# kangzf/GraphEmbedding

Hardware: AMD Instinct MI355X
Metric: graph-pairs/sec (Siamese fwd+bwd), AIDS700 all-pairs @ 1/2/4/8 MI355X (higher is better)
Workload: dtype f32; 1 GPU; AIDS700nef all-pairs (700 graphs, 490,000 ordered pairs), default 5-layer Siamese GCN-NTN, dropout 0.1; global_batch=490000, n_max=10, d_in=29, records=f32 Â, 896 B/pair, order=class, inputs=records resident in HBM, parallelism=dp1, adam=in the gradient reduction's launch (sg_train_step)

## Files before the change

graphembedding_amd/csrc/sg_fast.hip:

```cpp
#include <type_traits>

#include "sg_plan.h"
#include "sg_mfma.h"

int sg_num_cus();

namespace {

using namespace sgk;

constexpr int FH1 = 32, FH2 = 16, FK = 10;
constexpr int TS1 = 36;
constexpr int TS2 = 20;
constexpr int W1S = 20;
constexpr int W1TS = 36;
__device__ __forceinline__ void mfma_fence() { __builtin_amdgcn_sched_barrier(0); }
constexpr int MAXW = 8;

struct FastArgs {
  const uint8_t *recs;
  const int32_t *order;
  const int32_t *cls;
  float cw[4];
  int xw[8];
  int xw_even;
  int64_t n_pairs;
  int64_t pair_offset;
  int rw4h;
  int rec_bf16;
  const float *params;
  const float *y_stats;
  float *s_out;
  float *slab;
  float *ntn;
  uint32_t key;
  const uint64_t *seed_dev;
  const float *ad_bp;
  float *ad_out;
  float ad_lr, ad_b1, ad_b2, ad_wd;
  uint32_t thr0, thr1, thr2, thr4;
  float ik0, ik1, ik2, ik4;
  float yeta;
  float inv_batch;
  int d_in, n_params;
  int shared_floats, wave_floats;
  int oW0, ob0, oW1, ob1, oWd, obd, oW, oV, oU, obn;
  int oWa;
  int src_store, G;
  const float *sadj;
  const int32_t *stypes, *sn, *spairs;
  int64_t grid_base;
  const float *slabels;
  int32_t *status;
};

template <int D>
__device__ __forceinline__ uint4 fast_store_word(const FastArgs &A, int p, int w4, int lane) {
  int g0, g1;
  if (A.spairs) {
    g0 = A.spairs[2 * (int64_t)p];
    g1 = A.spairs[2 * (int64_t)p + 1];
  } else {
    const int64_t q = A.grid_base + p;
    g0 = (int)(q / A.G);
    g1 = (int)(q - (int64_t)g0 * A.G);
  }
  const bool ok = (unsigned)g0 < (unsigned)A.G && (unsigned)g1 < (unsigned)A.G;
  if (!ok && lane == 0 && A.status) atomicExch(A.status, (int32_t)SG_ERR_ARG);
  constexpr int NN = D * D;
  uint32_t v[4];
#pragma unroll
  for (int k = 0; k < 4; ++k) {
    const int w = 4 * w4 + k;
    uint32_t x = 0u;
    if (ok) {
      if (w < 2 * NN) {
        const int s = w >= NN;
        x = __float_as_uint(A.sadj[(size_t)(s ? g1 : g0) * NN + (w - s * NN)]);
      } else if (w < 2 * NN + 2 * D) {
        const int t = w - 2 * NN, s = t >= D;
        x = (uint32_t)A.stypes[(size_t)(s ? g1 : g0) * D + (t - s * D)];
      } else if (w == 2 * NN + 2 * D) {
        x = (uint32_t)A.sn[g0];
      } else if (w == 2 * NN + 2 * D + 1) {
        x = (uint32_t)A.sn[g1];
      } else if (w == 2 * NN + 2 * D + 2) {
        x = __float_as_uint(A.slabels ? A.slabels[p] : 0.f);
      } else if (w == 2 * NN + 2 * D + 3) {
        x = (uint32_t)p;
      }
    }
    v[k] = x;
  }
  return uint4{v[0], v[1], v[2], v[3]};
}

constexpr int WAS = 17;

template <int D, bool AVG = false, bool ATT = false>
struct FastLds {
  static constexpr int DN = AVG ? FH2 : D, WR = AVG ? 16 : 12, VS = 34;
  static_assert(2 * DN <= VS, "V row");
  static constexpr int RW = 2 * D * D + 2 * D + 4;
  static constexpr int REC = 0;
  static constexpr int TILE = REC + RW;
  static constexpr int X = TILE + 2 * 16 * TS1;
  static constexpr int GE = X + 48;
  static constexpr int TMP = GE + 32;
  static constexpr int GU = TMP + 32;
  static constexpr int GT = GU + 32;
  static int wave_floats(int, bool bwd) {
    return bwd ? GT + 2 * 16 * TS2 : X + 48 + (AVG ? 32 : 0) + (ATT ? 64 : 0);
  }
  static int shared_floats(int d_in) {
    return (d_in + 1) * FH1 + 2 * DN * FK * WR + FK * VS + FH1 * W1S + FH2 * W1TS +
           2 * 3 * 64 * 4 + (ATT ? FH2 * WAS : 0);
  }
};


template <int D, bool AVG = false, bool ATT = false>
struct FlushSlots {
  static constexpr int DN = FastLds<D, AVG>::DN, RN = (DN + 3) / 4;
  static constexpr int NWS = AVG ? 0 : RN * DN, NVS = AVG ? 0 : 2 * RN;
  static constexpr int NS = 8 + 16 + NWS + NVS + 3 + 5 + (ATT ? 4 : 0);
};

template <int D, bool AVG, bool ATT>
__device__ __forceinline__ int fast_param(const FastArgs &A, int s, int l) {
  constexpr int DN = FastLds<D, AVG>::DN, RN = (DN + 3) / 4;
  constexpr int NWS = FlushSlots<D, AVG>::NWS, NVS = FlushSlots<D, AVG>::NVS;
  const int g = l >> 4, j = l & 15;
  if (s < 8) return A.oW1 + (16 * (s >> 2) + 4 * g + (s & 3)) * FH2 + j;
  s -= 8;
  if (s < 16) {
    const int ty = 16 * (s >> 3) + 4 * g + (s & 3);
    return ty < A.d_in ? A.oW0 + ty * FH1 + 16 * ((s >> 2) & 1) + j : -1;
  }
  s -= 16;
  if (s < NWS) {
    const int a = 4 * (s / DN) + g, b = s % DN;
    return (a < DN && j < FK) ? A.oW + (a * DN + b) * FK + j : -1;
  }
  s -= NWS;
  if (s < NVS) {
    const int a = 4 * (s % RN) + g;
    return (a < DN && j < FK) ? A.oV + j * 2 * DN + (s >= RN ? DN : 0) + a : -1;
  }
  s -= NVS;
  switch (s) {
    case 0: return (!AVG && g == 0 && j < FK) ? A.obn + j : -1;
    case 1: return (g == 0 && j < FK) ? A.oU + j : -1;
    case 2: return l == 0 ? A.n_params : -1;
    case 3: return g == 0 ? A.ob0 + j : -1;
    case 4: return g == 0 ? A.ob0 + 16 + j : -1;
    case 5: return g == 0 ? A.ob1 + j : -1;
    case 6: return (!AVG && g == 0) ? A.oWd + j : -1;
    case 7: return (!AVG && l == 0) ? A.obd : -1;
    default: break;
  }
  s -= 8;
  return (ATT && s < 4) ? A.oWa + (4 * s + g) * FH2 + j : -1;
}

__device__ __forceinline__ f2 pfma(f2 a, f2 b, f2 c) { return __builtin_elementwise_fma(a, b, c); }

__device__ __forceinline__ float sg_tanh(float z) {
  return 1.f - 2.f * __builtin_amdgcn_rcpf(__expf(2.f * z) + 1.f);
}
__device__ __forceinline__ float sg_sigmoid(float z) {
  return __builtin_amdgcn_rcpf(1.f + __expf(-z));
}

__device__ __forceinline__ void xsum_pair(float &a, float &b) {
  const auto r = __builtin_amdgcn_permlane16_swap(__float_as_uint(a), __float_as_uint(b), false,
                                                  false);
  const float s = __uint_as_float(r[0]) + __uint_as_float(r[1]);
  const auto q = __builtin_amdgcn_permlane32_swap(__float_as_uint(s), __float_as_uint(s), false,
                                                  false);
  const float t = __uint_as_float(q[0]) + __uint_as_float(q[1]);
  const auto z = __builtin_amdgcn_permlane16_swap(__float_as_uint(t), __float_as_uint(t), false,
                                                  false);
  a = __uint_as_float(z[0]);
  b = __uint_as_float(z[1]);
}

#ifdef SG_FAST_TIMING
constexpr int kTimeWaves = 4096;
__device__ unsigned long long sg_fast_times[kTimeWaves * 5];
#define SG_STAMP(slot, val)                                                        \
  do {                                                                             \
    const int tw_ = blockIdx.x * (blockDim.x >> 6) + (threadIdx.x >> 6);            \
    if ((threadIdx.x & 63) == 0 && tw_ < kTimeWaves) sg_fast_times[tw_ * 5 + (slot)] = (val); \
  } while (0)
#else
#define SG_STAMP(slot, val) do {} while (0)
#endif

template <int D, bool BWD, bool ALIGNED, bool INTENDED, bool AVG, bool SRC, bool ATT>
// ... 77 lines not shown
        for (int c = 0; c < 4; ++c)
          if (wt[c] > 0.f && fr[c] > bf) {
            bf = fr[c];
            bc = c;
          }
        wc[bc] += 1;
        fr[bc] = -2.f;
      }
      if (align) {
#pragma unroll
        for (int c = 0; c < 4; ++c) wc[c] *= 2;
      }
      int cum = 0;
#pragma unroll
      for (int c = 0; c < 4; ++c) {
        if (cwave < 0 && pos < cum + wc[c]) {
          const int nc = cb[c + 1] - cb[c];
          cwave = c;
          const int q = nc / wc[c], r = nc - q * wc[c];
          if (q >= 64 && A.xw_even) {
            const int k = pos - cum;
            if ((uint64_t)(uint32_t)nc * (uint32_t)wc[c] < (1ull << 32)) {
              cs0 = cb[c] + __builtin_amdgcn_readfirstlane(
                                (int)(((uint32_t)nc * (uint32_t)k) / (uint32_t)wc[c]));
              cs1 = cb[c] + __builtin_amdgcn_readfirstlane(
                                (int)(((uint32_t)nc * (uint32_t)(k + 1)) / (uint32_t)wc[c]));
            } else {
              cs0 = cb[c] + (int)((int64_t)nc * k / wc[c]);
              cs1 = cb[c] + (int)((int64_t)nc * (k + 1) / wc[c]);
            }
          } else if (q >= 64) {
            auto F = [&](int x) -> int64_t {
              const int xb = (x >> 3) & 7;
              int64_t pre = 0, tot = 0;
#pragma unroll
              for (int i = 0; i < 8; ++i) {
                tot += A.xw[i];
                pre += i < xb ? A.xw[i] : 0;
              }
              return (int64_t)(x >> 6) * 8 * tot + 8 * pre + (int64_t)(x & 7) * A.xw[xb];
            };
            const int64_t f0 = F(cum), span = F(cum + wc[c]) - f0;
            cs0 = cb[c] + (int)((int64_t)nc * (F(pos) - f0) / span);
            cs1 = cb[c] + (int)((int64_t)nc * (F(pos + 1) - f0) / span);
          } else {
            int k;
            if (align) {
              k = ((gw & 4) == 0 ? 0 : wc[c] >> 1) + ((pos - cum) >> 1);
            } else {
              auto old_below = [](int x) -> int { return (x >> 3) * 4 + min(x & 7, 4); };
              const int end = cum + wc[c];
              const int n_old = old_below(end) - old_below(cum);
              k = (gw & 4) == 0 ? old_below(gw) - old_below(cum)
                                : n_old + (gw - old_below(gw)) - (cum - old_below(cum));
            }
            cs0 = cb[c] + k * q + min(k, r);
            cs1 = cs0 + q + (k < r ? 1 : 0);
          }
        }
        cum += wc[c];
      }
    }
  }
  const bool cls_mode = cwave >= 0;
  const int qend = cls_mode ? cs1 : npairs;
  auto slot_of = [&](int r) -> int {
    if (cls_mode) return cs0 + r;
    return r * stride + ((ord != nullptr && (r & 1)) ? stride - 1 - gw : gw);
  };
  auto load_ord = [&](int r0) -> int {
    const int s = slot_of(r0 + l);
    return s < qend ? ord[s] : 0;
  };
  auto ord_at = [&](int v, int lane) -> int {
    const int x = __builtin_amdgcn_readlane(v, lane);
    return x < 0 ? 0 : (x >= npairs ? npairs - 1 : x);
  };
  int ordA = 0, ordB = 0;
  if (ord) {
    ordA = load_ord(0);
    ordB = load_ord(64);
  }

  float *sW0 = smem;
  float *sWa = sW0 + (d_in + 1) * FH1;
  float *sWb = sWa + DN * FK * WR;
  float *sV = sWb + DN * FK * WR;
  float *sW1 = sV + FK * VS;
  float *sW1T = sW1 + FH1 * W1S;
  uint4 *sW1B = (uint4 *)(sW1T + FH2 * W1TS);
  float *sWat = (float *)(sW1B + 2 * 3 * 64);
  float *W = smem + A.shared_floats + wv * A.wave_floats;
  float *sRec = W + L::REC;
  float *sT = W + L::TILE;
  float *sX = W + L::X;

#pragma unroll
  for (int k = 0; k < 8; ++k) {
    const int i = k * bdx + tid;
    if (i < nprm) stg[i] = stv[k];
  }
  for (int i = 8 * bdx + tid; i < nprm; i += bdx) stg[i] = prm[i];
  int q = slot_of(0);
  int p = (ord && q < qend) ? ord_at(ordA, 0) : q;
  const int rw4h = A.rw4h;
  constexpr int ADJ4 = D * D / 4;
  uint4 pre[NREC];
#pragma unroll
  for (int c = 0; c < NREC; ++c) {
    const int w4 = l + 64 * c;
    pre[c] = (q < qend && w4 < rw4h)
                 ? (SRC ? fast_store_word<D>(A, p, w4, l)
                                : ((const uint4 *)(A.recs + (size_t)p * (size_t)rw4h * 16u))[w4])
                 : uint4{0u, 0u, 0u, 0u};
  }
  __syncthreads();
  if (ad_blk) {
    double ss = 0.0;
    for (int i = l; i < nprm; i += 64) {
      const double t = (double)stg[i];
      ss += t * t;
    }
#pragma unroll
    for (int o = 32; o > 0; o >>= 1) ss += __shfl_xor(ss, o);
    if (l == 0) {
      A.ad_out[0] = A.ad_lr * sqrtf(1.f - ad_b2p) / (1.f - ad_b1p);
      A.ad_out[1] = ad_b1p * A.ad_b1;
      A.ad_out[2] = ad_b2p * A.ad_b2;
      A.ad_out[3] = (float)((double)A.ad_wd * 0.5 * ss);
    }
  }
  auto wa_src = [&](int i, bool tr) -> float {
    const int x = i / (FK * WR), rem = i - x * FK * WR, k = rem / WR, y = rem - k * WR;
    return y < DN ? stg[A.oW + (tr ? (y * DN + x) : (x * DN + y)) * FK + k] : 0.f;
  };
  auto v_src = [&](int i) -> float {
    const int k = i / VS, c = i - k * VS;
    return c < 2 * DN ? stg[A.oV + k * 2 * DN + c] : 0.f;
  };
  constexpr int NWA = DN * FK * WR, KWA = (NWA + 511) / 512, NVT = FK * VS, KV = (NVT + 511) / 512;
  static_assert(FH1 * FH2 == 512, "one W1 element per thread of a 512-thread block");
  const int nw0 = (d_in + 1) * FH1;
  if (bdx == 512 && nw0 <= 3 * 512) {
    float r0[3], ra[KWA], rb[KWA], rv[KV];
#pragma unroll
    for (int k = 0; k < 3; ++k) {
      const int i = min(tid + 512 * k, nw0 - 1);
      r0[k] = i < d_in * FH1 ? stg[A.oW0 + i] : 0.f;
    }
#pragma unroll
    for (int k = 0; k < KWA; ++k) {
      const int i = min(tid + 512 * k, NWA - 1);
      ra[k] = wa_src(i, false);
      rb[k] = wa_src(i, true);
    }
#pragma unroll
    for (int k = 0; k < KV; ++k) rv[k] = v_src(min(tid + 512 * k, NVT - 1));
    const float w1 = stg[A.oW1 + tid];
#pragma unroll
    for (int k = 0; k < 3; ++k)
      if (tid + 512 * k < nw0) sW0[tid + 512 * k] = r0[k] * (A.ik0 * A.ik1);
#pragma unroll
    for (int k = 0; k < KWA; ++k)
      if (tid + 512 * k < NWA) {
        sWa[tid + 512 * k] = ra[k];
        sWb[tid + 512 * k] = rb[k];
      }
#pragma unroll
    for (int k = 0; k < KV; ++k)
      if (tid + 512 * k < NVT) sV[tid + 512 * k] = rv[k];
    sW1[(tid / FH2) * W1S + tid % FH2] = w1 * A.ik1;
    sW1T[(tid % FH2) * W1TS + tid / FH2] = w1;
  } else {
    for (int i = tid; i < nw0; i += bdx)
      sW0[i] = i < d_in * FH1 ? stg[A.oW0 + i] * (A.ik0 * A.ik1) : 0.f;
    for (int i = tid; i < NWA; i += bdx) {
      sWa[i] = wa_src(i, false);
      sWb[i] = wa_src(i, true);
    }
    for (int i = tid; i < NVT; i += bdx) sV[i] = v_src(i);
    for (int i = tid; i < FH1 * FH2; i += bdx) {
      const float w = stg[A.oW1 + i];
      sW1[(i / FH2) * W1S + i % FH2] = w * A.ik1;
      sW1T[(i % FH2) * W1TS + i / FH2] = w;
    }
  }
  for (int i = tid; i < 2 * 3 * 64; i += blockDim.x) {
    const int t = i / 192, term = (i / 64) % 3, ln = i & 63;
    const int f = 16 * t + (ln & 15), k0 = 4 * (ln >> 4);
    const float *wr = stg + A.oW1 + f * FH2 + k0;
    uint32_t h01, m01, l01, h23, m23, l23;
    split3(wr[0] * A.ik1, wr[1] * A.ik1, h01, m01, l01);
    split3(wr[2] * A.ik1, wr[3] * A.ik1, h23, m23, l23);
    sW1B[i] = term == 0 ? uint4{h01, h23, h01, h23}
                        : (term == 1 ? uint4{m01, m23, h01, h23} : uint4{l01, l23, m01, m23});
  }
  if constexpr (ATT)
    for (int i = tid; i < FH2 * FH2; i += blockDim.x) sWat[(i >> 4) * WAS + (i & 15)] = stg[A.oWa + i];
  const int j_ = tid & 15;
  const float b0v0 = stg[A.ob0 + j_] * A.ik1, b0v1 = stg[A.ob0 + 16 + j_] * A.ik1;
  const float b1v = stg[A.ob1 + j_];
  const float wdv = AVG ? 0.f : stg[A.oWd + j_] * A.ik2;
  const float bd = AVG ? 0.f : stg[A.obd];
  const bool kv = j_ < FK;
  const int kc = kv ? j_ : FK - 1;
  const float Uk = kv ? stg[A.oU + kc] : 0.f;
  const float bnk = kv ? stg[A.obn + kc] : 0.f;
  float usum = 0.f;
#pragma unroll
  for (int k = 0; k < FK; ++k) usum += stg[A.oU + k];
  __syncthreads();
  static_assert((2 * 16 * TS1) % 4 == 0, "D1 tiles in float4s");
  for (int i = l; i < 2 * 16 * TS1 / 4; i += 64) ((f4 *)sT)[i] = f4{0.f, 0.f, 0.f, 0.f};
  if (l < 48) sX[l] = 0.f;
  SG_STAMP(1, __builtin_amdgcn_s_memrealtime());

  const float *w1bp = sW1T + j * W1TS + 8 * g;
  const int ri = j & 3, ni = 4 * ri + (j >> 2);
  int afo[2][3];
#pragma unroll
  for (int s = 0; s < 2; ++s)
#pragma unroll
    for (int q = 0; q < 3; ++q) {
      const int c = 4 * q + g;
      afo[s][q] = (ri < 3 && ni < D && c < D) ? L::REC + s * D * D + ni * D + c : L::X + 47;
    }
  const int jp = (j >> 1) & 1, jr = j - 2 * jp;
  const float *sTp = sT + jp * 16 * TS1 + jr * TS1 + 8 * g;
  int tyo[3];
#pragma unroll
  for (int r = 0; r < 3; ++r) tyo[r] = 2 * D * D + (4 * r + g < D ? 4 * r + g : 0);

  f4 gw1[2] = {f4{0.f, 0.f, 0.f, 0.f}, f4{0.f, 0.f, 0.f, 0.f}};
  f4 gw0[2][2] = {{f4{0.f, 0.f, 0.f, 0.f}, f4{0.f, 0.f, 0.f, 0.f}},
                  {f4{0.f, 0.f, 0.f, 0.f}, f4{0.f, 0.f, 0.f, 0.f}}};
  float gb0a0 = 0.f, gb0a1 = 0.f, gb1a = 0.f, gwda = 0.f, gbda = 0.f;
  constexpr int RW_ = AVG ? 1 : RN, DW_ = AVG ? 1 : DN;
  f2 gWn[RW_][(DW_ + 1) / 2];
  float gVa[RW_], gVb[RW_];
#pragma unroll
  for (int r = 0; r < RW_; ++r) {
    gVa[r] = gVb[r] = 0.f;
#pragma unroll
    for (int b = 0; b < (DW_ + 1) / 2; ++b) gWn[r][b] = f2{0.f, 0.f};
  }
  float gbn = 0.f, gUa = 0.f, lossa = 0.f;
  float gwa[4] = {0.f, 0.f, 0.f, 0.f};
  const float ybar = (BWD && !ALIGNED) ? A.y_stats[0] : 0.f;

  constexpr int PRIO_PERIOD = 3, PRIO_YOUNG = 2;
  int it = 0;
  const int young = wv >> 2;
  auto pair_loop = [&](auto CLSc) __attribute__((always_inline)) {
  constexpr int CLS = decltype(CLSc)::value;
  for (; q < qend; ++it) {
    const int yturn = (int)((unsigned)((it % PRIO_PERIOD) - PRIO_YOUNG) >> 31);
    __builtin_amdgcn_s_setprio(0);
    if ((yturn ^ young) == 0) __builtin_amdgcn_s_setprio(1);
    sg_wsync();
    if (A.rec_bf16) {
#pragma unroll
      for (int c = 0; c < NREC; ++c) {
        const int w4 = l + 64 * c;
        const uint4 v = pre[c];
        if (w4 < ADJ4) {
          f4 lo = {__uint_as_float(v.x << 16), __uint_as_float(v.x & 0xFFFF0000u),
                   __uint_as_float(v.y << 16), __uint_as_float(v.y & 0xFFFF0000u)};
          f4 hi = {__uint_as_float(v.z << 16), __uint_as_float(v.z & 0xFFFF0000u),
                   __uint_as_float(v.w << 16), __uint_as_float(v.w & 0xFFFF0000u)};
          ((f4 *)sRec)[2 * w4] = lo;
          ((f4 *)sRec)[2 * w4 + 1] = hi;
        } else if (w4 < rw4h) {
          ((uint4 *)sRec)[w4 + ADJ4] = v;
        }
      }
    } else {
#pragma unroll
      for (int c = 0; c < NREC; ++c) {
        const int w4 = l + 64 * c;
        if (w4 < RW4) ((uint4 *)sRec)[w4] = pre[c];
      }
    }
    sg_wsync();
    const int pcur = p;
    {
      const int qn = slot_of(it + 1);
      int pn = qn;
      if (ord) {
        const int rl = (it + 1) & 63;
        if (rl == 0) {
          ordA = ordB;
          ordB = load_ord(it + 65);
        }
        pn = qn < qend ? ord_at(ordA, rl) : 0;
      }
#pragma unroll
      for (int c = 0; c < NREC; ++c) {
        const int w4 = l + 64 * c;
        if (qn < qend && w4 < rw4h)
          pre[c] = SRC
                       ? fast_store_word<D>(A, pn, w4, l)
                       : ((const uint4 *)(A.recs + (size_t)pn * (size_t)rw4h * 16u))[w4];
      }
      q = qn;
      p = pn;
    }
    const int *ty = (const int *)sRec;
    int N0 = __builtin_amdgcn_readfirstlane(((const int *)sRec)[2 * D * D + 2 * D]);
    int N1 = __builtin_amdgcn_readfirstlane(((const int *)sRec)[2 * D * D + 2 * D + 1]);
    N0 = N0 < 0 ? 0 : (N0 > D ? D : N0);
    N1 = N1 < 0 ? 0 : (N1 > D ? D : N1);
    const uint32_t pk = sg_pair_key(key, (uint32_t)(A.pair_offset + pcur));
    const uint32_t pk1 = pk ^ lb1, pk2 = pk ^ lb2;

    uint32_t km, km4;
    uint32_t m4;
    {
      const int e = l & 15;
      const bool hi = l >= 16;
      const uint32_t h = sg_hash(pk, hi ? NL : 0u, (uint32_t)e);
      const uint32_t thr = hi ? thr4s : thr0s;
      const bool p0 = (hi && AVG) || e < N0, p1 = (hi && AVG) || e < N1;
      const uint64_t b0 = __ballot((l < 32) & p0 & ((h & 0xFFFFu) < thr));
      const uint64_t b1 = __ballot((l < 32) & p1 & ((h >> 16) < thr));
      const uint32_t m0 = (uint32_t)(b0 & 0xFFFFu) | ((uint32_t)(b1 & 0xFFFFu) << 16);
      m4 = (uint32_t)((b0 >> 16) & 0xFFFFu) | ((uint32_t)b1 & 0xFFFF0000u);
      km = m0 >> g;
      km4 = m4 >> g;
    }
    const float invn0 = N0 > 0 ? 1.f / (float)N0 : 0.f, invn1 = N1 > 0 ? 1.f / (float)N1 : 0.f;

    auto body = [&](auto K0c, auto K1c) __attribute__((always_inline)) {
      constexpr int K0 = decltype(K0c)::value, K1 = decltype(K1c)::value;
      float af[2][3];
      f4 p1[2][2];
      uint32_t tys[2];
#pragma unroll
      for (int s = 0; s < 2; ++s) {
        const int KS = s ? K1 : K0;
#pragma unroll
        for (int q = 0; q < 3; ++q) af[s][q] = q < KS ? W[afo[s][q]] : 0.f;
        f4 z0[2];
        uint32_t tp = 0u;
#pragma unroll
        for (int r = 0; r < 3; ++r) {
          if (r < KS) {
            uint32_t t_ = (uint32_t)ty[tyo[r] + s * D];
            t_ = min(t_, (uint32_t)(d_in - 1));
            const uint32_t k0 = (km >> (16 * s + 4 * r)) & 1u;
            const uint32_t tk = k0 ? t_ : 63u;
            tp |= tk << (6 * r);
            const float *w0 = sW0 + (k0 ? t_ : (uint32_t)d_in) * FH1 + j;
            z0[0][r] = w0[0];
            z0[1][r] = w0[16];
          } else {
            tp |= 63u << (6 * r);
            z0[0][r] = z0[1][r] = 0.f;
          }
        }
        tys[s] = tp;
        mfma_fence();
#pragma unroll
        for (int t = 0; t < 2; ++t) {
          const float bb = t ? b0v1 : b0v0;
          f4 acc = {bb, bb, bb, bb};
#pragma unroll
          for (int q = 0; q < KS; ++q) acc = mfma4(af[s][q], z0[t][q], acc);
          p1[s][t] = acc;
        }
        mfma_fence();
      }
#pragma unroll
      for (int r = 0; r < 3; ++r) {
#pragma unroll
        for (int t = 0; t < 2; ++t) {
          if (r < K0 || r < K1) {
            const uint32_t h = sg_mix(pk1 ^ ((1u << 26) | (uint32_t)(128 * r + 16 * t)));
#pragma unroll
            for (int s = 0; s < 2; ++s) {
              float *T = sT + s * 16 * TS1 + (4 * g + r) * TS1 + 16 * t + j;
              if (r < (s ? K1 : K0)) {
                const uint32_t d = s ? (h >> 16) : (h & 0xFFFFu);
                const float v = relu_bits(p1[s][t][r]);
                *T = d < A.thr1 ? v : 0.f;
              } else {
                *T = 0.f;
              }
            }
          } else {
            sT[(4 * g + r) * TS1 + 16 * t + j] = 0.f;
            sT[16 * TS1 + (4 * g + r) * TS1 + 16 * t + j] = 0.f;
          }
        }
      }
      sg_wsync();
      constexpr bool PACK = K0 == 2 && K1 == 2;
      f4 h2[2];
      if constexpr (PACK) {
        const f4 lo = *(const f4 *)sTp, hi = *(const f4 *)(sTp + 4);
        const f4 wlo = *(const f4 *)w1bp, whi = *(const f4 *)(w1bp + 4);
        f4 z1 = {0.f, 0.f, 0.f, 0.f};
        mfma_fence();
#pragma unroll
        for (int q = 0; q < 4; ++q) z1 = mfma4(lo[q], wlo[q], z1);
#pragma unroll
        for (int q = 0; q < 4; ++q) z1 = mfma4(hi[q], whi[q], z1);
#pragma unroll
        for (int s = 0; s < 2; ++s) {
          f4 acc = {b1v, b1v, b1v, b1v};
          acc = mfma4(af[s][0], z1[2 * s], acc);
          acc = mfma4(af[s][1], z1[2 * s + 1], acc);
          h2[s] = acc;
        }
        mfma_fence();
      } else {
#pragma unroll
        for (int s = 0; s < 2; ++s) {
          const int KS = s ? K1 : K0;
          const float *T = sT + s * 16 * TS1 + j * TS1 + 8 * g;
          const f4 lo = *(const f4 *)T, hi = *(const f4 *)(T + 4);
          const f4 wlo = *(const f4 *)w1bp, whi = *(const f4 *)(w1bp + 4);
          f4 z1 = {0.f, 0.f, 0.f, 0.f};
          mfma_fence();
#pragma unroll
          for (int q = 0; q < 4; ++q) z1 = mfma4(lo[q], wlo[q], z1);
#pragma unroll
          for (int q = 0; q < 4; ++q) z1 = mfma4(hi[q], whi[q], z1);
          f4 acc = {b1v, b1v, b1v, b1v};
#pragma unroll
          for (int q = 0; q < KS; ++q) acc = mfma4(af[s][q], z1[q], acc);
          h2[s] = acc;
          mfma_fence();
        }
      }
      float xo[2][RN], d2[2][3];
      uint32_t kb = 0u;
      float hA[2] = {0.f, 0.f};
      float att[2][3] = {{0.f, 0.f, 0.f}, {0.f, 0.f, 0.f}};
      if constexpr (ATT) {
        float *sTmp = W + L::TMP;
        float part[2] = {0.f, 0.f};
#pragma unroll
        for (int s2 = 0; s2 < 2; ++s2) {
          const int KS = s2 ? K1 : K0, Ns = s2 ? N1 : N0;
#pragma unroll
          for (int r = 0; r < KS; ++r) part[s2] += (4 * r + g < Ns) ? h2[s2][r] : 0.f;
        }
        xsum_pair(part[0], part[1]);
#pragma unroll
        for (int s2 = 0; s2 < 2; ++s2)
          if (g == 0) sTmp[16 * s2 + j] = part[s2] * (s2 ? invn1 : invn0);
        sg_wsync();
        float hp[2];
// ... 413 lines not shown
  if (cls_mode) {
    if (cwave == 0) pair_loop(std::integral_constant<int, 0>{});
    else if (cwave == 1) pair_loop(std::integral_constant<int, 1>{});
    else if (cwave == 2) pair_loop(std::integral_constant<int, 2>{});
    else pair_loop(std::integral_constant<int, 3>{});
  } else {
    pair_loop(std::integral_constant<int, -1>{});
  }

  SG_STAMP(2, __builtin_amdgcn_s_memrealtime());
  SG_STAMP(4, (unsigned long long)it | ((unsigned long long)(cwave + 1) << 32));
  if (!BWD) return;
  constexpr int NS = FlushSlots<D, AVG, ATT>::NS;
  {
    gb0a0 = xsum32(xsum16(gb0a0));
    gb0a1 = xsum32(xsum16(gb0a1));
    gb1a = xsum32(xsum16(gb1a));
    gwda = xsum32(xsum16(gwda)) * A.ik2;
    gbda = xsum32(xsum16(gbda));
  }
  float *F = smem;
  __syncthreads();
  {
    float *Fw = F + (size_t)wv * NS * 64 + l;
    int s = 0;
#pragma unroll
    for (int t = 0; t < 2; ++t)
#pragma unroll
      for (int r = 0; r < 4; ++r) Fw[64 * s++] = gw1[t][r];
#pragma unroll
    for (int tau = 0; tau < 2; ++tau)
#pragma unroll
      for (int t = 0; t < 2; ++t)
#pragma unroll
        for (int r = 0; r < 4; ++r) Fw[64 * s++] = gw0[tau][t][r] * A.ik0;
    if constexpr (!AVG) {
#pragma unroll
      for (int r = 0; r < RN; ++r)
#pragma unroll
        for (int b = 0; b < DN; ++b) Fw[64 * s++] = gWn[r][b >> 1][b & 1];
#pragma unroll
      for (int r = 0; r < RN; ++r) Fw[64 * s++] = gVa[r];
#pragma unroll
      for (int r = 0; r < RN; ++r) Fw[64 * s++] = gVb[r];
    }
    Fw[64 * s++] = gbn;
    Fw[64 * s++] = gUa;
    Fw[64 * s++] = lossa;
    Fw[64 * s++] = gb0a0;
    Fw[64 * s++] = gb0a1;
    Fw[64 * s++] = gb1a;
    Fw[64 * s++] = gwda;
    Fw[64 * s++] = gbda;
    if constexpr (ATT) {
#pragma unroll
      for (int i = 0; i < 4; ++i) Fw[64 * s++] = gwa[i];
    }
  }
  __syncthreads();
  float *dst = A.slab + (size_t)blockIdx.x * (size_t)(A.n_params + 1);
  for (int s = wv; s < NS; s += nw) {
    const int prm_i = fast_param<D, AVG, ATT>(A, s, l);
    float acc = 0.f;
    for (int w = 0; w < nw; ++w) acc += F[((size_t)w * NS + s) * 64 + l];
    if (prm_i >= 0) dst[prm_i] = acc;
  }
  SG_STAMP(3, __builtin_amdgcn_s_memrealtime());
}

struct FastCfg {
  int D;
  int waves;
  int blocks;
  size_t lds;
  int shared_floats, wave_floats;
};

template <int D, bool AVG, bool ATT>
FastCfg fast_cfg_t(int d_in, int n_params, int64_t n_pairs, bool bwd) {
  FastCfg c;
  c.D = D;
  using LL = FastLds<D, AVG, ATT>;
  using FS = FlushSlots<D, AVG, ATT>;
  c.shared_floats = LL::shared_floats(d_in);
  c.wave_floats = LL::wave_floats(d_in, bwd);
  const int wcap = bwd ? MAXW : 2 * MAXW;
  int best = 1, best_res = 0;
  const char *ev = getenv("SG_FAST_WAVES");
  const int force = ev ? atoi(ev) : 0;
  for (int nw = 1; nw <= MAXW; ++nw) {
    if (force > 0 && nw != force) continue;
    const size_t lds = (size_t)(c.shared_floats + nw * c.wave_floats) * 4u;
    if (lds > 163840u) break;
    if (bwd && (size_t)nw * FS::NS * 256u > 163840u) break;
    int per_cu = (int)(163840u / lds);
    int res = per_cu * nw;
    if (res > wcap) res = wcap;
    if (res > best_res || (res == best_res && nw > best)) {
      best = nw;
      best_res = res;
    }
  }
  c.waves = best;
  c.lds = (size_t)(c.shared_floats + best * c.wave_floats) * 4u;
  int per_cu = (int)(163840u / c.lds);
  if (per_cu > wcap / best) per_cu = wcap / best;
  if (per_cu < 1) per_cu = 1;
  const size_t fl = bwd ? (size_t)best * FS::NS * 64u * 4u : 0u;
  const size_t stage = (size_t)(c.shared_floats + n_params) * 4u;
  const size_t need = fl > stage ? fl : stage;
  if (need > c.lds) {
    c.lds = need;
    per_cu = (int)(163840u / c.lds);
  }
  const int64_t want = (n_pairs + best - 1) / best;
  const int64_t cap = (int64_t)sg_num_cus() * per_cu;
  c.blocks = (int)(want < cap ? (want > 0 ? want : 1) : cap);
  return c;
}

template <int D, bool BWD, bool ALIGNED, bool INTENDED, bool AVG, bool SRC, bool ATT>
void launch_one(const FastCfg &c, const FastArgs &A, hipStream_t st) {
  const void *fn = (const void *)sg_fast_kernel<D, BWD, ALIGNED, INTENDED, AVG, SRC, ATT>;
  if (c.lds > 65536u)
    (void)hipFuncSetAttribute(fn, hipFuncAttributeMaxDynamicSharedMemorySize, (int)c.lds);
  hipLaunchKernelGGL((sg_fast_kernel<D, BWD, ALIGNED, INTENDED, AVG, SRC, ATT>), dim3(c.blocks),
                     dim3(64 * c.waves), c.lds, st, A);
}

template <int D, bool AVG, bool SRC, bool ATT>
void launch_fast_src(const FastCfg &c, bool bwd, bool aligned, bool intended,
                     const FastArgs &A, hipStream_t st) {
  if (!bwd) {
    if (intended) launch_one<D, false, false, true, AVG, SRC, ATT>(c, A, st);
    else launch_one<D, false, false, false, AVG, SRC, ATT>(c, A, st);
  } else if (aligned) {
    if (intended) launch_one<D, true, true, true, AVG, SRC, ATT>(c, A, st);
    else launch_one<D, true, true, false, AVG, SRC, ATT>(c, A, st);
  } else {
    if (intended) launch_one<D, true, false, true, AVG, SRC, ATT>(c, A, st);
    else launch_one<D, true, false, false, AVG, SRC, ATT>(c, A, st);
  }
}

template <int D, bool AVG, bool ATT = false>
void launch_fast(const FastCfg &c, bool bwd, bool aligned, bool intended,
                 const FastArgs &A, hipStream_t st) {
  if (A.src_store) launch_fast_src<D, AVG, true, ATT>(c, bwd, aligned, intended, A, st);
  else launch_fast_src<D, AVG, false, ATT>(c, bwd, aligned, intended, A, st);
}

}

static bool fast_pool_shape(const sg_model_t *m, const SgGenPlan &P) {
  if (m->num_layers != 4) return false;
  const sg_layer_t *Ly = m->layers;
  if (Ly[0].kind != SG_GCN || !Ly[0].sparse_inputs || Ly[0].output_dim != FH1 ||
      Ly[0].act != SG_ACT_RELU || !Ly[0].bias)
    return false;
  if (Ly[1].kind != SG_GCN || Ly[1].input_dim != FH1 || Ly[1].output_dim != FH2 ||
      Ly[1].act != SG_ACT_IDENTITY || !Ly[1].bias)
    return false;
  if (Ly[2].kind != SG_AVERAGE && !(Ly[2].kind == SG_ATTENTION && Ly[2].input_dim == FH2))
    return false;
  if (Ly[3].kind != SG_NTN || Ly[3].input_dim != FH2 || Ly[3].output_dim != FK ||
      Ly[3].act != SG_ACT_RELU || !Ly[3].bias)
    return false;
// ... 173 lines not shown
  A.ob0 = P.L[0].offB;
  A.oW1 = P.L[1].offW;
  A.ob1 = P.L[1].offB;
  A.oWd = avg ? -1 : P.L[2].offW;
  A.obd = avg ? -1 : P.L[2].offB;
  A.oWa = att ? P.L[2].offW : -1;
  A.oW = P.offW;
  A.oV = P.offV;
  A.oU = P.offU;
  A.obn = P.offB;
  const bool aligned = m->loss_mode == SG_LOSS_ALIGNED;
  const bool intended = m->ntn_mode == SG_NTN_INTENDED;
  if (avg && bwd && !ntn) return SG_ERR_ARG;
#ifdef SG_FAST_ATT_TU
  if (!att) return SG_ERR_UNSUPPORTED;
  if (D == 12) launch_fast<12, true, true>(c, bwd, aligned, intended, A, stream);
  else launch_fast<10, true, true>(c, bwd, aligned, intended, A, stream);
#else
  if (att) return SG_ERR_UNSUPPORTED;
  if (avg) {
    if (D == 12) launch_fast<12, true>(c, bwd, aligned, intended, A, stream);
    else launch_fast<10, true>(c, bwd, aligned, intended, A, stream);
  } else {
    if (D == 12) launch_fast<12, false>(c, bwd, aligned, intended, A, stream);
    else launch_fast<10, false>(c, bwd, aligned, intended, A, stream);
  }
#endif
  if (avg && bwd) {
    const int rc = sg_ntn_wgrad_run(ntn, n_pairs, FH2, P.offW, P.offV, P.offB, P.n_params + 1,
                                    slab, c.blocks, stream, true);
    if (rc != SG_OK) return rc;
  }
  if (blocks_out) *blocks_out = c.blocks;
  return hipGetLastError() == hipSuccess ? SG_OK : SG_ERR_HIP;
}

#ifdef SG_FAST_ATT_TU
int sg_fast_att_run(const sg_model_t *m, const SgGenPlan &P, bool bwd, const void *recs,
                    const int32_t *order, int64_t n_pairs, int64_t pair_offset,
                    int64_t batch_total, const float *params, uint64_t seed,
                    const float *y_stats, float *s_out, float *slab, float *ntn, int *blocks_out,
                    hipStream_t stream, const uint64_t *seed_dev, const sg_pair_source_t *src,
                    const int32_t *class_start, const SgAdamPre *adam_pre) {
  return fast_run_impl(m, P, bwd, recs, order, n_pairs, pair_offset, batch_total, params, seed,
                       y_stats, s_out, slab, ntn, blocks_out, stream, seed_dev, src, class_start,
                       adam_pre);
}
#else
int sg_fast_att_run(const sg_model_t *m, const SgGenPlan &P, bool bwd, const void *recs,
                    const int32_t *order, int64_t n_pairs, int64_t pair_offset,
                    int64_t batch_total, const float *params, uint64_t seed,
                    const float *y_stats, float *s_out, float *slab, float *ntn, int *blocks_out,
                    hipStream_t stream, const uint64_t *seed_dev, const sg_pair_source_t *src,
                    const int32_t *class_start, const SgAdamPre *adam_pre);

int sg_fast_supported(const sg_model_t *m, const SgGenPlan &P) {
  if (getenv("SG_DISABLE_FAST")) return 0;
  return fast_shape(m, P) ? 1 : 0;
}

int64_t sg_fast_slab_floats(const SgGenPlan &P, int64_t n_pairs) {
  FastCfg c = fast_cfg(P, n_pairs, true);
  return (int64_t)c.blocks * (P.n_params + 1);
}

int sg_fast_needs_ntn(const SgGenPlan &P) { return plan_avg(P) ? 1 : 0; }

int sg_fast_run(const sg_model_t *m, const SgGenPlan &P, bool bwd, const void *recs,
                const int32_t *order, int64_t n_pairs, int64_t pair_offset, int64_t batch_total,
                const float *params, uint64_t seed, const float *y_stats, float *s_out,
                float *slab, float *ntn, int *blocks_out, hipStream_t stream,
                const uint64_t *seed_dev, const sg_pair_source_t *src,
                const int32_t *class_start, const SgAdamPre *adam_pre) {
  if (plan_att(P))
    return sg_fast_att_run(m, P, bwd, recs, order, n_pairs, pair_offset, batch_total, params,
                           seed, y_stats, s_out, slab, ntn, blocks_out, stream, seed_dev, src,
                           class_start, adam_pre);
  return fast_run_impl(m, P, bwd, recs, order, n_pairs, pair_offset, batch_total, params, seed,
                       y_stats, s_out, slab, ntn, blocks_out, stream, seed_dev, src, class_start,
                       adam_pre);
}
#endif

#if defined(SG_FAST_TIMING) && !defined(SG_FAST_ATT_TU)
extern "C" int sg_fast_timing_fetch(unsigned long long *host, int n) {
  if (n > kTimeWaves * 5) n = kTimeWaves * 5;
  return hipMemcpyFromSymbol(host, HIP_SYMBOL(sg_fast_times), (size_t)n * 8u, 0,
                             hipMemcpyDeviceToHost) == hipSuccess ? n : -1;
}
#endif
```

graphembedding_amd/csrc/sg_mfma.h:

```cpp
#pragma once
#include <hip/hip_runtime.h>
#include <stdint.h>

namespace sgk {

typedef float f4 __attribute__((ext_vector_type(4)));
typedef float f2 __attribute__((ext_vector_type(2)));

__device__ __forceinline__ f4 mfma4(float a, float b, f4 c) {
  return __builtin_amdgcn_mfma_f32_16x16x4f32(a, b, c, 0, 0, 0);
}

typedef __bf16 bf8 __attribute__((ext_vector_type(8)));
typedef __bf16 bf2v __attribute__((ext_vector_type(2)));

__device__ __forceinline__ uint32_t pk_bf16(float a, float b) {
  const bf2v v = {(__bf16)a, (__bf16)b};
  return __builtin_bit_cast(uint32_t, v);
}
__device__ __forceinline__ uint32_t hi16x2(uint32_t a, uint32_t b) {
  return __builtin_amdgcn_perm(b, a, 0x07060302u);
}
#ifndef SG_SPLIT_PK
#define SG_SPLIT_PK 0
#endif
__device__ __forceinline__ void split3(float x0, float x1, uint32_t &h, uint32_t &m, uint32_t &l) {
  const uint32_t u0 = __float_as_uint(x0), u1 = __float_as_uint(x1);
  h = hi16x2(u0, u1);
#if SG_SPLIT_PK
  const f2 r = f2{x0, x1} - f2{__uint_as_float(u0 & 0xFFFF0000u), __uint_as_float(u1 & 0xFFFF0000u)};
  const float r0 = r.x, r1 = r.y;
#else
  const float r0 = x0 - __uint_as_float(u0 & 0xFFFF0000u), r1 = x1 - __uint_as_float(u1 & 0xFFFF0000u);
#endif
  const uint32_t v0 = __float_as_uint(r0), v1 = __float_as_uint(r1);
  m = hi16x2(v0, v1);
#if SG_SPLIT_PK
  const f2 t = f2{r0, r1} - f2{__uint_as_float(v0 & 0xFFFF0000u), __uint_as_float(v1 & 0xFFFF0000u)};
  const float s0 = t.x, s1 = t.y;
#else
  const float s0 = r0 - __uint_as_float(v0 & 0xFFFF0000u), s1 = r1 - __uint_as_float(v1 & 0xFFFF0000u);
#endif
  l = hi16x2(__float_as_uint(s0), __float_as_uint(s1));
}
__device__ __forceinline__ f4 mfbf(uint4 a, uint4 b, f4 c) {
  return __builtin_amdgcn_mfma_f32_16x16x32_bf16(__builtin_bit_cast(bf8, a),
                                                  __builtin_bit_cast(bf8, b), c, 0, 0, 0);
}
typedef short s4 __attribute__((ext_vector_type(4)));
__device__ __forceinline__ f4 mfbf16(uint2 a, uint2 b, f4 c) {
  return __builtin_amdgcn_mfma_f32_16x16x16bf16_1k(__builtin_bit_cast(s4, a),
                                                    __builtin_bit_cast(s4, b), c, 0, 0, 0);
}

__device__ __forceinline__ float relu_bits(float x) {
  return __int_as_float(max(__float_as_int(x), 0));
}

template <int CTRL>
__device__ __forceinline__ float dpp(float v) {
  return __builtin_bit_cast(float, __builtin_amdgcn_mov_dpp(__builtin_bit_cast(int, v), CTRL,
                                                            0xF, 0xF, true));
}


__device__ __forceinline__ float xsum16(float x) {
  const auto r = __builtin_amdgcn_permlane16_swap(__float_as_uint(x), __float_as_uint(x), false,
                                                  false);
  return __uint_as_float(r[0]) + __uint_as_float(r[1]);
}
__device__ __forceinline__ float xsum32(float x) {
  const auto r = __builtin_amdgcn_permlane32_swap(__float_as_uint(x), __float_as_uint(x), false,
                                                  false);
  return __uint_as_float(r[0]) + __uint_as_float(r[1]);
}

__device__ __forceinline__ float row_sum16(float v) {
  v += dpp<0xB1>(v);
  v += dpp<0x4E>(v);
  v += dpp<0x141>(v);
  v += dpp<0x140>(v);
  return v;
}

template <int N>
__device__ __forceinline__ void row_sum16_n(float (&v)[N]) {
#pragma unroll
  for (int i = 0; i < N; ++i) asm("" : "+v"(v[i]));
#pragma unroll
  for (int i = 0; i < N; ++i) v[i] += dpp<0xB1>(v[i]);
#pragma unroll
  for (int i = 0; i < N; ++i) v[i] += dpp<0x4E>(v[i]);
#pragma unroll
  for (int i = 0; i < N; ++i) v[i] += dpp<0x141>(v[i]);
#pragma unroll
  for (int i = 0; i < N; ++i) v[i] += dpp<0x140>(v[i]);
}

}
```

Baseline: 580.7 million graph-pairs/s.

## Compute first GCN layer with split-bf16 MFMA instead of f32 MFMA

The first-layer W0 table in LDS is replaced by pre-split bf16 hi/mid/lo parts packed as uint4 per element. Each activation is split on the fly, so the f32 16x16x4 MFMAs become 16x16x32 bf16 MFMAs that emulate f32 precision with multiple bf16 products. The unused sW1 table is dropped and the sW1B build is limited to backward kernels, which shrinks the shared LDS footprint. In exchange the W0 table grows fourfold in LDS, more VALU work is spent splitting values, and rounding differs slightly from true f32.

New measurement: 579.9 million graph-pairs/s. Within noise of the previous version (-0.1%).

```diff
diff --git a/graphembedding_amd/csrc/sg_fast.hip b/graphembedding_amd/csrc/sg_fast.hip
--- a/graphembedding_amd/csrc/sg_fast.hip
+++ b/graphembedding_amd/csrc/sg_fast.hip
@@ -12,7 +12,6 @@
 constexpr int FH1 = 32, FH2 = 16, FK = 10;
 constexpr int TS1 = 36;
 constexpr int TS2 = 20;
-constexpr int W1S = 20;
 constexpr int W1TS = 36;
 __device__ __forceinline__ void mfma_fence() { __builtin_amdgcn_sched_barrier(0); }
 constexpr int MAXW = 8;
@@ -112,9 +111,9 @@
   static int wave_floats(int, bool bwd) {
     return bwd ? GT + 2 * 16 * TS2 : X + 48 + (AVG ? 32 : 0) + (ATT ? 64 : 0);
   }
-  static int shared_floats(int d_in) {
-    return (d_in + 1) * FH1 + 2 * DN * FK * WR + FK * VS + FH1 * W1S + FH2 * W1TS +
-           2 * 3 * 64 * 4 + (ATT ? FH2 * WAS : 0);
+  static int shared_floats(int d_in, bool bwd) {
+    return 4 * (d_in + 1) * FH1 + 2 * DN * FK * WR + FK * VS + FH2 * W1TS +
+           (bwd ? 2 * 3 * 64 * 4 : 0) + (ATT ? FH2 * WAS : 0);
   }
 };
 
@@ -358,14 +357,13 @@
     ordB = load_ord(64);
   }
 
-  float *sW0 = smem;
-  float *sWa = sW0 + (d_in + 1) * FH1;
+  uint4 *sW0S = (uint4 *)smem;
+  float *sWa = smem + 4 * (d_in + 1) * FH1;
   float *sWb = sWa + DN * FK * WR;
   float *sV = sWb + DN * FK * WR;
-  float *sW1 = sV + FK * VS;
-  float *sW1T = sW1 + FH1 * W1S;
+  float *sW1T = sV + FK * VS;
   uint4 *sW1B = (uint4 *)(sW1T + FH2 * W1TS);
-  float *sWat = (float *)(sW1B + 2 * 3 * 64);
+  float *sWat = (float *)(sW1B + (BWD ? 2 * 3 * 64 : 0));
   float *W = smem + A.shared_floats + wv * A.wave_floats;
   float *sRec = W + L::REC;
   float *sT = W + L::TILE;
@@ -435,7 +433,7 @@
     const float w1 = stg[A.oW1 + tid];
 #pragma unroll
     for (int k = 0; k < 3; ++k)
-      if (tid + 512 * k < nw0) sW0[tid + 512 * k] = r0[k] * (A.ik0 * A.ik1);
+      if (tid + 512 * k < nw0) sW0S[tid + 512 * k] = az0_b_parts(r0[k] * (A.ik0 * A.ik1));
 #pragma unroll
     for (int k = 0; k < KWA; ++k)
       if (tid + 512 * k < NWA) {
@@ -445,11 +443,10 @@
 #pragma unroll
     for (int k = 0; k < KV; ++k)
       if (tid + 512 * k < NVT) sV[tid + 512 * k] = rv[k];
-    sW1[(tid / FH2) * W1S + tid % FH2] = w1 * A.ik1;
     sW1T[(tid % FH2) * W1TS + tid / FH2] = w1;
   } else {
     for (int i = tid; i < nw0; i += bdx)
-      sW0[i] = i < d_in * FH1 ? stg[A.oW0 + i] * (A.ik0 * A.ik1) : 0.f;
+      sW0S[i] = az0_b_parts(i < d_in * FH1 ? stg[A.oW0 + i] * (A.ik0 * A.ik1) : 0.f);
     for (int i = tid; i < NWA; i += bdx) {
       sWa[i] = wa_src(i, false);
       sWb[i] = wa_src(i, true);
@@ -457,11 +454,10 @@
     for (int i = tid; i < NVT; i += bdx) sV[i] = v_src(i);
     for (int i = tid; i < FH1 * FH2; i += bdx) {
       const float w = stg[A.oW1 + i];
-      sW1[(i / FH2) * W1S + i % FH2] = w * A.ik1;
       sW1T[(i % FH2) * W1TS + i / FH2] = w;
     }
   }
-  for (int i = tid; i < 2 * 3 * 64; i += blockDim.x) {
+  for (int i = tid; BWD && i < 2 * 3 * 64; i += blockDim.x) {
     const int t = i / 192, term = (i / 64) % 3, ln = i & 63;
     const int f = 16 * t + (ln & 15), k0 = 4 * (ln >> 4);
     const float *wr = stg + A.oW1 + f * FH2 + k0;
@@ -616,7 +612,7 @@
         const int KS = s ? K1 : K0;
 #pragma unroll
         for (int q = 0; q < 3; ++q) af[s][q] = q < KS ? W[afo[s][q]] : 0.f;
-        f4 z0[2];
+        uint4 zb[2][3];
         uint32_t tp = 0u;
 #pragma unroll
         for (int r = 0; r < 3; ++r) {
@@ -626,25 +622,25 @@
             const uint32_t k0 = (km >> (16 * s + 4 * r)) & 1u;
             const uint32_t tk = k0 ? t_ : 63u;
             tp |= tk << (6 * r);
-            const float *w0 = sW0 + (k0 ? t_ : (uint32_t)d_in) * FH1 + j;
-            z0[0][r] = w0[0];
-            z0[1][r] = w0[16];
+            const uint4 *w0 = sW0S + (k0 ? t_ : (uint32_t)d_in) * FH1 + j;
+            zb[0][r] = w0[0];
+            zb[1][r] = w0[16];
           } else {
             tp |= 63u << (6 * r);
-            z0[0][r] = z0[1][r] = 0.f;
           }
         }
         tys[s] = tp;
-        mfma_fence();
+        uint4 aa[3];
+#pragma unroll
+        for (int q = 0; q < KS; ++q) aa[q] = az0_a_parts(af[s][q]);
 #pragma unroll
         for (int t = 0; t < 2; ++t) {
           const float bb = t ? b0v1 : b0v0;
           f4 acc = {bb, bb, bb, bb};
 #pragma unroll
-          for (int q = 0; q < KS; ++q) acc = mfma4(af[s][q], z0[t][q], acc);
+          for (int q = 0; q < KS; ++q) acc = mfbf(aa[q], zb[t][q], acc);
           p1[s][t] = acc;
         }
-        mfma_fence();
       }
 #pragma unroll
       for (int r = 0; r < 3; ++r) {
@@ -1224,7 +1220,7 @@
   c.D = D;
   using LL = FastLds<D, AVG, ATT>;
   using FS = FlushSlots<D, AVG, ATT>;
-  c.shared_floats = LL::shared_floats(d_in);
+  c.shared_floats = LL::shared_floats(d_in, bwd);
   c.wave_floats = LL::wave_floats(d_in, bwd);
   const int wcap = bwd ? MAXW : 2 * MAXW;
   int best = 1, best_res = 0;
@@ -1564,8 +1560,12 @@
 }
 #endif
 
-#if defined(SG_FAST_TIMING) && !defined(SG_FAST_ATT_TU)
+#if defined(SG_FAST_TIMING)
+#ifdef SG_FAST_ATT_TU
+extern "C" int sg_fast_att_timing_fetch(unsigned long long *host, int n) {
+#else
 extern "C" int sg_fast_timing_fetch(unsigned long long *host, int n) {
+#endif
   if (n > kTimeWaves * 5) n = kTimeWaves * 5;
   return hipMemcpyFromSymbol(host, HIP_SYMBOL(sg_fast_times), (size_t)n * 8u, 0,
                              hipMemcpyDeviceToHost) == hipSuccess ? n : -1;
diff --git a/graphembedding_amd/csrc/sg_mfma.h b/graphembedding_amd/csrc/sg_mfma.h
--- a/graphembedding_amd/csrc/sg_mfma.h
+++ b/graphembedding_amd/csrc/sg_mfma.h
@@ -46,6 +46,21 @@
 __device__ __forceinline__ f4 mfbf(uint4 a, uint4 b, f4 c) {
   return __builtin_amdgcn_mfma_f32_16x16x32_bf16(__builtin_bit_cast(bf8, a),
                                                   __builtin_bit_cast(bf8, b), c, 0, 0, 0);
+}
+__device__ __forceinline__ uint4 az0_a_parts(float x) {
+  const uint32_t u = __float_as_uint(x);
+  const float r = x - __uint_as_float(u & 0xFFFF0000u);
+  const uint32_t v = __float_as_uint(r);
+  const uint32_t w = __float_as_uint(r - __uint_as_float(v & 0xFFFF0000u));
+  return uint4{hi16x2(u, u), hi16x2(u, w), hi16x2(v, v), hi16x2(v, w)};
+}
+__device__ __forceinline__ uint4 az0_b_parts(float x) {
+  const uint32_t u = __float_as_uint(x);
+  const float r = x - __uint_as_float(u & 0xFFFF0000u);
+  const uint32_t v = __float_as_uint(r);
+  const uint32_t w = __float_as_uint(r - __uint_as_float(v & 0xFFFF0000u));
+  const uint32_t hm = hi16x2(u, v);
+  return uint4{hm, hi16x2(w, u), hm, hi16x2(w, v)};
 }
 typedef short s4 __attribute__((ext_vector_type(4)));
 __device__ __forceinline__ f4 mfbf16(uint2 a, uint2 b, f4 c) {
```
